# ConsenSys/wittgenstein

Hardware: NVIDIA H100
Metric: simulated-ms/sec, GSFSignature 65,536 nodes (higher is better)
Workload: dtype u64 bitmaps / int32

## Files before the change

wittgenstein_b200/csrc/wtg_cuda.cu:

```cuda
#include <cuda_runtime.h>
#include <unistd.h>

#include <cstdio>
#include <cstdlib>
#include <stdexcept>
#include <string>
#include <vector>

#include "wtg_engine.hpp"

namespace wtg {

#define CUDA_OK(x)                                                                                       \
  do {                                                                                                   \
    cudaError_t e_ = (x);                                                                                \
    if (e_ != cudaSuccess) throw std::runtime_error(std::string("CUDA: ") + cudaGetErrorString(e_) + " at " #x); \
  } while (0)

constexpr int SCAN_THREADS = 256;
constexpr int SCAN_ITEMS = 4;
constexpr int SCAN_TILE = SCAN_THREADS * SCAN_ITEMS;

__global__ void k_begin(Dev d, int mode) {
  if (threadIdx.x >= 32) return;
// ... 424 lines not shown
  if (warp >= 4) return;
  const int gw = blk * 4 + warp, nw = nBlk * 4;
  CoopWarp c;
  for (int k = gw; k < cnt; k += nw) xBuildAll(d, c, k, d.allTmp + (size_t)gw * d.N, hist[warp]);
}

constexpr int MS_SUB = 256;
constexpr int MS_ROUNDS = MS_SUB / 32;
__device__ __forceinline__ void msZero(int* hist, int ring, int warps) {
  for (int i = threadIdx.x * 4; i < warps * ring; i += blockDim.x * 4) *reinterpret_cast<int4*>(hist + i) = make_int4(0, 0, 0, 0);
}
__device__ __forceinline__ void msWarpHistogram(const Dev& d, int* hw, int g0, int G, int tick, int lane, int (&tg)[MS_ROUNDS]) {
#pragma unroll
  for (int r = 0; r < MS_ROUNDS; ++r) {
    int g = g0 + r * 32 + lane;
    tg[r] = g < G ? d.newTarget[g] : -1;
  }
#pragma unroll
  for (int r = 0; r < MS_ROUNDS; ++r)
    if (tg[r] >= 0) atomicAdd(&hw[tg[r] - tick], 1);
}
__global__ void __launch_bounds__(256) k_ms_count(Dev d) {
  extern __shared__ int msHist[];
  if (d.ctl->error) return;
  const int blk = blockIdx.x, nBlk = gridDim.x;
  const int G = d.ctl->totalSlots, tick = d.ctl->tick, ring = d.ring;
  const int W = d.msWarps, CH = W * MS_SUB;
  const int nChunks = (G + CH - 1) / CH;
  const int warp = threadIdx.x >> 5, lane = threadIdx.x & 31;
  for (int ch = blk; ch < nChunks; ch += nBlk) {
    msZero(msHist, ring, W);
    __syncthreads();
    int tg[MS_ROUNDS];
    msWarpHistogram(d, msHist + warp * ring, ch * CH + warp * MS_SUB, G, tick, lane, tg);
    __syncthreads();
    int* row = d.msCount + (size_t)ch * ring;
    for (int b = threadIdx.x; b < ring; b += blockDim.x) {
      int tot = 0;
      for (int w = 0; w < W; ++w) tot += msHist[w * ring + b];
      row[b] = tot;
    }
    __syncthreads();
  }
}
__global__ void k_ms_scan(Dev d) {
  if (d.ctl->error) return;
  const int blk = blockIdx.x, nBlk = gridDim.x;
  int G = d.ctl->totalSlots, tick = d.ctl->tick, ring = d.ring;
  const int CH = d.msWarps * MS_SUB;
  int nChunks = (G + CH - 1) / CH;
  if (nChunks == 0) return;
  for (int b = blk * blockDim.x + threadIdx.x; b < ring; b += nBlk * blockDim.x) {
    int slot = (tick + b) & (ring - 1);
    int run = d.bucketCount[slot];
    for (int ch0 = 0; ch0 < nChunks; ch0 += 8) {
      int v[8];
#pragma unroll
      for (int k = 0; k < 8; ++k) v[k] = ch0 + k < nChunks ? d.msCount[(size_t)(ch0 + k) * ring + b] : 0;
#pragma unroll
      for (int k = 0; k < 8; ++k)
        if (ch0 + k < nChunks) {
          d.msCount[(size_t)(ch0 + k) * ring + b] = run;
          run += v[k];
        }
    }
    if (run > d.bcap) {
      setError(d, ERR_BUCKET_OVERFLOW, tick + b);
      run = d.bcap;
    }
    d.bucketCount[slot] = run;
  }
}
__global__ void __launch_bounds__(256) k_ms_scatter(Dev d) {
  extern __shared__ int msHist[];
  if (d.ctl->error) return;
  const int blk = blockIdx.x, nBlk = gridDim.x;
  const int G = d.ctl->totalSlots, tick = d.ctl->tick, ring = d.ring;
  const int W = d.msWarps, CH = W * MS_SUB;
  const int nChunks = (G + CH - 1) / CH;
  const int warp = threadIdx.x >> 5, lane = threadIdx.x & 31;
  int* base = msHist + warp * ring;
  CoopWarp cw;
  for (int ch = blk; ch < nChunks; ch += nBlk) {
    msZero(msHist, ring, W);
    __syncthreads();
    const int g0 = ch * CH + warp * MS_SUB;
    int tg[MS_ROUNDS];
    msWarpHistogram(d, base, g0, G, tick, lane, tg);
    __syncthreads();
    const int* row = d.msCount + (size_t)ch * ring;
    for (int b = threadIdx.x; b < ring; b += blockDim.x) {
      int run = row[b];
      for (int w = 0; w < W; ++w) {
        int c = msHist[w * ring + b];
        msHist[w * ring + b] = run;
        run += c;
      }
    }
    __syncthreads();
#pragma unroll
    for (int r = 0; r < MS_ROUNDS; ++r) {
      int g = g0 + r * 32 + lane;
      int t = tg[r];
      int pos = cw.claim(base, t - tick, t >= 0);
      if (t >= 0) {
        if (pos < d.bcap) {
          const int4* src = reinterpret_cast<const int4*>(d.newEv + g);
          int4* dst = reinterpret_cast<int4*>(d.buckets + (size_t)(t & (ring - 1)) * (size_t)d.bcap + pos);
          int4 x = src[0], y = src[1];
          dst[0] = x;
          dst[1] = y;
          if (d.G > 1) d.bucketKey[(size_t)(t & (ring - 1)) * (size_t)d.bcap + pos] = orderKey((unsigned)d.ctl->xseq, (unsigned)g);
        }
        if (d.G > 1) d.newTarget[g] = -1;
      }
      __syncwarp();
    }
    __syncthreads();
  }
}

__global__ void k_free(Dev d) {
  if (d.ctl->error) return;
  const int blk = blockIdx.x, nBlk = gridDim.x;
  const int per = d.freeCap / ARENA_STRIPES;
  const int stripe = blk & (ARENA_STRIPES - 1);
  int cnt = d.ctl->freeCnt[stripe];
  if (cnt > per) cnt = per;
  const int sub = (blk >> 6) * blockDim.x + threadIdx.x;
  const int nsub = (nBlk >> 6) * blockDim.x;
  for (int j = sub; j < cnt; j += nsub) freeApply(d, stripe * per + j);
}

__global__ void k_gsf_init_nodes(Dev d) {
  int n = d.n0 + blockIdx.x * blockDim.x + threadIdx.x;
  if (n < d.n0 + d.nLoc) gsfInitNodeBody(d, n);
}
__global__ void k_rng_candidates(Dev d, u64 s0, u64 count, u64 chunk, int maxBound, u64* out, int* outCount, int cap) {
  u64 t = (u64)blockIdx.x * blockDim.x + threadIdx.x;
  u64 start = t * chunk;
  if (start >= count) return;
  u64 len = start + chunk <= count ? chunk : count - start;
  rngCandidateChunk(d, s0, start, len, maxBound, out, outCount, cap);
}
template <class PeerT>
__global__ void k_gsf_shuffle(Dev d, int l, u64 s0, const int* liveRank, const u64* rejOrd, int nRej) {
  int n = d.n0 + blockIdx.x * blockDim.x + threadIdx.x;
  if (n < d.n0 + d.nLoc) gsfShuffleLevel<PeerT>(d, n, l, s0, liveRank, rejOrd, nRej);
}

class CudaBackend : public Backend {
 public:
  cudaStream_t st = nullptr;
  int devId = 0;
  void bind() const { cudaSetDevice(devId); }
  int sms = 132;
  int smemOptin = 0;
  cudaGraphExec_t tickGraph = nullptr;
  const void* graphFor = nullptr;
  bool useGraph = true;
  long long launches = 0;
  long long graphKernels = 0;
  cudaEvent_t tm0 = nullptr, tm1 = nullptr;
  enum ProfSlot { P_BEGIN, P_COND_SCAN, P_DISPATCH_COUNT, P_SCAN_PARTIAL, P_EXCHANGE, P_SCAN_FINAL, P_DISPATCH_SCATTER, P_NODE,
                  P_EMIT, P_MS_COUNT, P_MS_SCAN, P_MS_SCATTER, P_FREE, P_END, P_COND_SCORE, P_COND_SELECT, NK };
  bool profiling = false;
  std::vector<cudaEvent_t> evPool;
  std::vector<int> evKernel;
  size_t evUsed = 0;
  double profMs[NK] = {};
  long long profCnt[NK] = {};
  const char* profNames[NK] = {"k_begin", "k_cond_scan", "k_dispatch_count", "k_scan_partial", "k_exchange", "k_scan_final",
                               "k_dispatch_scatter", "k_node", "k_emit", "k_ms_count", "k_ms_scan", "k_ms_scatter", "k_free",
                               "k_end", "k_cond_score", "k_cond_select"};

  explicit CudaBackend(int requested = -1) {
    int dev = 0;
    const char* e = std::getenv("LOCAL_RANK");
    int cnt = 0;
    CUDA_OK(cudaGetDeviceCount(&cnt));
    if (cnt == 0) throw std::runtime_error("no CUDA device");
    if (e) dev = std::atoi(e) % cnt;
    const char* e2 = std::getenv("WTG_DEVICE");
    if (e2) dev = std::atoi(e2) % cnt;
    if (requested >= 0) {
      if (requested >= cnt) throw std::invalid_argument("CUDA device " + std::to_string(requested) + " does not exist");
      dev = requested;
    }
    CUDA_OK(cudaSetDevice(dev));
    devId = dev;
    cudaDeviceProp p;
    CUDA_OK(cudaGetDeviceProperties(&p, dev));
    sms = p.multiProcessorCount;
    CUDA_OK(cudaStreamCreateWithFlags(&st, cudaStreamNonBlocking));
    CUDA_OK(cudaDeviceGetAttribute(&smemOptin, cudaDevAttrMaxSharedMemoryPerBlockOptin, dev));
    CUDA_OK(cudaFuncSetAttribute(k_ms_count, cudaFuncAttributeMaxDynamicSharedMemorySize, smemOptin));
    CUDA_OK(cudaFuncSetAttribute(k_ms_scatter, cudaFuncAttributeMaxDynamicSharedMemorySize, smemOptin));
    const char* g = std::getenv("WTG_NO_GRAPH");
    if (g && g[0] == '1') useGraph = false;
  }
  ~CudaBackend() override {
    for (void* q : ipcOpened) cudaIpcCloseMemHandle(q);
    if (tickGraph) cudaGraphExecDestroy(tickGraph);
    if (st) cudaStreamDestroy(st);
  }
  void* alloc(size_t bytes) override {
    bind();
    void* p = nullptr;
    cudaError_t e = cudaMalloc(&p, bytes);
    if (e != cudaSuccess) throw std::runtime_error("cudaMalloc of " + std::to_string(bytes) + " bytes failed: " + cudaGetErrorString(e));
    CUDA_OK(cudaMemsetAsync(p, 0, bytes, st));
    return p;
  }
  void release(void* p) override { cudaFree(p); }
  int deviceId() const override { return devId; }
  void exportShared(void* p, unsigned char* handle) override {
    bind();
    std::memset(handle, 0, 128);
    cudaIpcMemHandle_t ih;
    CUDA_OK(cudaIpcGetMemHandle(&ih, p));
    static_assert(sizeof(ih) == 64, "cudaIpcMemHandle_t");
    std::memcpy(handle, &ih, 64);
    long long pid = (long long)getpid();
    std::memcpy(handle + 64, &pid, 8);
    std::memcpy(handle + 72, &p, sizeof(p));
    std::memcpy(handle + 80, &devId, 4);
  }
  std::vector<void*> ipcOpened;
  void* importShared(const unsigned char* handle) override {
    bind();
    long long pid;
    void* p;
    int dev;
    std::memcpy(&pid, handle + 64, 8);
    std::memcpy(&p, handle + 72, sizeof(p));
    std::memcpy(&dev, handle + 80, 4);
    if (pid == (long long)getpid()) {
      if (dev != devId) {
        int can = 0;
        CUDA_OK(cudaDeviceCanAccessPeer(&can, devId, dev));
        if (!can) throw std::runtime_error("GPU " + std::to_string(devId) + " cannot access GPU " + std::to_string(dev) + " (peer access)");
        cudaError_t e = cudaDeviceEnablePeerAccess(dev, 0);
        if (e != cudaSuccess && e != cudaErrorPeerAccessAlreadyEnabled) CUDA_OK(e);
        cudaGetLastError();
      }
      return p;
    }
    cudaIpcMemHandle_t ih;
    std::memcpy(&ih, handle, 64);
    void* q = nullptr;
    CUDA_OK(cudaIpcOpenMemHandle(&q, ih, cudaIpcMemLazyEnablePeerAccess));
    ipcOpened.push_back(q);
    return q;
  }
  void upload(void* dst, const void* src, size_t bytes) override {
    bind();
    CUDA_OK(cudaMemcpyAsync(dst, src, bytes, cudaMemcpyHostToDevice, st));
    CUDA_OK(cudaStreamSynchronize(st));
  }
  void download(void* dst, const void* src, size_t bytes) override {
    bind();
    CUDA_OK(cudaMemcpyAsync(dst, src, bytes, cudaMemcpyDeviceToHost, st));
    CUDA_OK(cudaStreamSynchronize(st));
  }
  void sync() override {
    bind();
    CUDA_OK(cudaStreamSynchronize(st));
    drainProfile();
  }
  void timerStart() override {
    bind();
    if (!tm0) {
      CUDA_OK(cudaEventCreate(&tm0));
      CUDA_OK(cudaEventCreate(&tm1));
    }
    CUDA_OK(cudaEventRecord(tm0, st));
  }
  double timerStopMs() override {
    bind();
    CUDA_OK(cudaEventRecord(tm1, st));
    CUDA_OK(cudaEventSynchronize(tm1));
    float ms = 0;
    CUDA_OK(cudaEventElapsedTime(&ms, tm0, tm1));
    return (double)ms;
  }
  void profileEnable(bool on) override {
    sync();
    profiling = on;
    if (on) {
      for (int i = 0; i < NK; ++i) {
        profMs[i] = 0;
        profCnt[i] = 0;
      }
    }
  }
  int profileRead(double* ms, long long* cnt, const char** names, int cap) override {
    sync();
    int k = 0;
    for (int i = 0; i < NK && k < cap; ++i, ++k) {
      ms[k] = profMs[i];
      cnt[k] = profCnt[i];
      names[k] = profNames[i];
    }
    return k;
  }
  void drainProfile() {
    for (size_t i = 0; i < evUsed; ++i) {
      float ms = 0;
      cudaEventElapsedTime(&ms, evPool[2 * i], evPool[2 * i + 1]);
      profMs[evKernel[i]] += ms;
      profCnt[evKernel[i]] += 1;
    }
    evUsed = 0;
  }
  void profBegin(int kid) {
    if (!profiling) return;
    if (evUsed * 2 + 2 > evPool.size()) {
      if (evUsed >= 8192) {
        CUDA_OK(cudaStreamSynchronize(st));
        drainProfile();
      } else {
        cudaEvent_t a, b;
        CUDA_OK(cudaEventCreate(&a));
        CUDA_OK(cudaEventCreate(&b));
        evPool.push_back(a);
        evPool.push_back(b);
        evKernel.push_back(0);
      }
    }
    evKernel[evUsed] = kid;
    CUDA_OK(cudaEventRecord(evPool[2 * evUsed], st));
  }
  void profEnd() {
    if (!profiling) return;
    CUDA_OK(cudaEventRecord(evPool[2 * evUsed + 1], st));
    ++evUsed;
  }

  void enqueueTick(const Dev& d, int mode) {
    const int wide = sms * 8;
    const size_t msSmem = (size_t)d.msWarps * d.ring * sizeof(int);
    if (mode != 3) {
      profBegin(P_BEGIN);
      k_begin<<<1, 32, 0, st>>>(d, mode);
      profEnd();
    }
    if ((d.proto == PROTO_GSF || d.proto == PROTO_HANDEL) && mode != 3) {
      const size_t smem8 = d.proto == PROTO_GSF ? (size_t)8 * (size_t)(d.qcap / 32) * sizeof(uint32_t) : 0;
      profBegin(P_COND_SCAN);
      k_cond_mark<<<(d.nLoc + 255) / 256, 256, 0, st>>>(d);
      k_cond_nodes<0><<<ARENA_STRIPES * 19, 256, 0, st>>>(d);
      profEnd();
      profBegin(P_COND_SCORE);
      k_cond_score<<<ARENA_STRIPES * 19, 256, 0, st>>>(d);
      profEnd();
      profBegin(P_COND_SELECT);
      k_cond_nodes<1><<<ARENA_STRIPES * 19, 256, smem8, st>>>(d);
      profEnd();
      launches += 4;
      if (d.proto == PROTO_HANDEL) {
        profBegin(P_SCAN_PARTIAL);
        k_scan_partial<<<wide, SCAN_THREADS, 0, st>>>(d, 2);
        profEnd();
        profBegin(P_SCAN_FINAL);
        k_scan_final<<<wide, SCAN_THREADS, 0, st>>>(d, 2);
        profEnd();
        if (d.G > 1) {
          profBegin(P_EXCHANGE);
          k_hpick_publish<<<sms, 256, 0, st>>>(d);
          k_x_sync<<<1, 32, 0, st>>>(d, 3);
          profEnd();
          profBegin(P_COND_SELECT);
          k_hpick_xcheck<<<sms, 256, 0, st>>>(d);
          k_hpick_xapply<<<sms, 256, 0, st>>>(d);
          profEnd();
          launches += 5;
        } else {
          profBegin(P_COND_SELECT);
          k_hpick_check<<<sms, 256, 0, st>>>(d);
          k_hpick_apply<<<sms, 256, 0, st>>>(d);
          profEnd();
          launches += 3;
        }
      }
    }
    if (mode != 2 && mode != 3) {
      profBegin(P_DISPATCH_COUNT);
      k_dispatch_count<<<wide, 256, 0, st>>>(d);
      profEnd();
      profBegin(P_SCAN_PARTIAL);
      k_scan_partial<<<wide, SCAN_THREADS, 0, st>>>(d, 0);
      profEnd();
      profBegin(P_SCAN_FINAL);
      k_scan_final<<<wide, SCAN_THREADS, 0, st>>>(d, 0);
      profEnd();
      profBegin(P_DISPATCH_SCATTER);
      k_dispatch_scatter<<<wide, 256, 0, st>>>(d);
      profEnd();
      profBegin(P_NODE);
      k_node_msgs<<<(d.nLoc + 255) / 256, 256, 0, st>>>(d);
      k_node_tasks<<<ARENA_STRIPES * 19, 256, 0, st>>>(d);
      if (d.proto == PROTO_CASPER) {
        k_casper_fixups<<<1, 32, 0, st>>>(d);
        launches += 1;
      }
      profEnd();
      launches += 6;
    }
    profBegin(P_SCAN_PARTIAL);
    k_scan_partial<<<wide, SCAN_THREADS, 0, st>>>(d, 1);
    profEnd();
    profBegin(P_SCAN_FINAL);
    k_scan_final<<<wide, SCAN_THREADS, 0, st>>>(d, 1);
    profEnd();
    if (d.G > 1) {
      profBegin(P_EXCHANGE);
      k_x1_publish<<<sms * 2, 256, 0, st>>>(d);
      k_x_sync<<<1, 32, 0, st>>>(d, 0);
      k_x1_totals<<<1, 1, 0, st>>>(d);
      k_x1_offsets<<<sms * 2, 256, 0, st>>>(d);
      profEnd();
      launches += 4;
    }
    profBegin(P_EMIT);
    if (d.shufCap > 0) {
      k_shuffle_check<<<ARENA_STRIPES * 4, 256, 0, st>>>(d);
      k_shuffle_serial<<<1, 1, 0, st>>>(d);
      launches += 2;
    }
    k_emit<<<ARENA_STRIPES * 16, 256, 0, st>>>(d);
    if (d.allCap > 0) {
      if (d.G > 1)
        k_x_all_publish<<<8, 128, 0, st>>>(d);
      else
        k_emit_all<<<d.allWarps / 4, 128, 0, st>>>(d);
      launches += 1;
    }
    profEnd();
    if (d.G > 1) {
      profBegin(P_EXCHANGE);
      k_x_sync<<<1, 32, 0, st>>>(d, 1);
      k_x2_ingest<<<sms * 4, 256, 0, st>>>(d);
      launches += 2;
      if (d.allCap > 0) {
        k_x_all_build<<<d.allWarps / 4, 128, 0, st>>>(d);
        launches += 1;
      }
      profEnd();
    }
    profBegin(P_MS_COUNT);
    k_ms_count<<<sms * 2, d.msWarps * 32, msSmem, st>>>(d);
    profEnd();
    profBegin(P_MS_SCAN);
    k_ms_scan<<<(d.ring + 127) / 128, 128, 0, st>>>(d);
    profEnd();
    profBegin(P_MS_SCATTER);
    k_ms_scatter<<<sms * 2, d.msWarps * 32, msSmem, st>>>(d);
    profEnd();
    const bool pooled = d.proto == PROTO_GSF || d.proto == PROTO_HANDEL;
    if (pooled) {
      profBegin(P_FREE);
      k_free<<<ARENA_STRIPES * 2, 256, 0, st>>>(d);
      profEnd();
    }
    profBegin(P_END);
    k_end<<<1, 1, 0, st>>>(d, mode);
    profEnd();
    launches += pooled ? 9 : 8;
  }
  void configure(const Dev& d) {
    const size_t msSmem = (size_t)d.msWarps * d.ring * sizeof(int);
    if (msSmem > (size_t)smemOptin) throw std::runtime_error("time ring too large for the multisplit's shared-memory histogram");
  }
  void tick(const Dev& d, int mode) override {
    bind();
    configure(d);
    enqueueTick(d, mode);
    CUDA_OK(cudaGetLastError());
  }
  void ticks(const Dev& d, int count) override {
    bind();
    configure(d);
    if (!useGraph || profiling || count < 4) {
      for (int i = 0; i < count; ++i) enqueueTick(d, 1);
      CUDA_OK(cudaGetLastError());
      return;
    }
    if (!tickGraph || graphFor != (const void*)d.ctl) {
      if (tickGraph) cudaGraphExecDestroy(tickGraph);
      cudaGraph_t g;
      long long before = launches;
      CUDA_OK(cudaStreamBeginCapture(st, cudaStreamCaptureModeThreadLocal));
      enqueueTick(d, 1);
      CUDA_OK(cudaStreamEndCapture(st, &g));
      graphKernels = launches - before;
      launches = before;
      CUDA_OK(cudaGraphInstantiate(&tickGraph, g, 0));
      cudaGraphDestroy(g);
      graphFor = (const void*)d.ctl;
    }
    for (int i = 0; i < count; ++i) CUDA_OK(cudaGraphLaunch(tickGraph, st));
    launches += graphKernels * count;
  }
  void gsfInitNodes(const Dev& d) override {
    bind();
    k_gsf_init_nodes<<<(d.nLoc + 255) / 256, 256, 0, st>>>(d);
    CUDA_OK(cudaGetLastError());
  }
  void rngCandidates(const Dev& d, unsigned long long s0, unsigned long long count, int maxBound,
                     std::vector<unsigned long long>& out) override {
    bind();
    const u64 chunk = 16384;
    u64 threads = (count + chunk - 1) / chunk;
    int cap = (int)std::min<u64>((u64)1 << 26, count / 1024 + (1 << 16));
    u64* dOut = nullptr;
    int* dCnt = nullptr;
    CUDA_OK(cudaMalloc(&dOut, (size_t)cap * sizeof(u64)));
    CUDA_OK(cudaMalloc(&dCnt, sizeof(int)));
    CUDA_OK(cudaMemsetAsync(dCnt, 0, sizeof(int), st));
    u64 blocks = (threads + 127) / 128;
    k_rng_candidates<<<(unsigned)blocks, 128, 0, st>>>(d, s0, count, chunk, maxBound, dOut, dCnt, cap);
    CUDA_OK(cudaGetLastError());
    int n = 0;
    CUDA_OK(cudaMemcpyAsync(&n, dCnt, sizeof(int), cudaMemcpyDeviceToHost, st));
    CUDA_OK(cudaStreamSynchronize(st));
    if (n > cap) {
      cudaFree(dOut);
      cudaFree(dCnt);
      throw std::runtime_error("rng candidate list overflow");
    }
    out.resize((size_t)n);
    if (n) CUDA_OK(cudaMemcpyAsync(out.data(), dOut, (size_t)n * sizeof(u64), cudaMemcpyDeviceToHost, st));
    CUDA_OK(cudaStreamSynchronize(st));
    cudaFree(dOut);
    cudaFree(dCnt);
  }
  void gsfShufflePeers(const Dev& d, unsigned long long s0, const int* liveRank, const unsigned long long* rejOrd, int nRej) override {
    bind();
    for (int l = d.L - 1; l >= 1; --l) {
      if (d.peerBits == 16)
        k_gsf_shuffle<uint16_t><<<(d.nLoc + 127) / 128, 128, 0, st>>>(d, l, s0, liveRank, rejOrd, nRej);
      else
        k_gsf_shuffle<uint32_t><<<(d.nLoc + 127) / 128, 128, 0, st>>>(d, l, s0, liveRank, rejOrd, nRej);
    }
    CUDA_OK(cudaGetLastError());
    CUDA_OK(cudaStreamSynchronize(st));
  }
};

Backend* makeBackend(int device) { return new CudaBackend(device); }
long long backendLaunches(Backend* b) { return static_cast<CudaBackend*>(b)->launches; }

}

#define WTG_API(name) wtg_##name
#include "wtg_capi.inl"
```

wittgenstein_b200/csrc/wtg_engine.hpp:

```cpp
#pragma once
#include <chrono>
#include <cstdio>
#include <functional>
#include <thread>
#include <cstdlib>
#include <cstring>
#include <memory>
#include <string>
#include <vector>

#include "wtg_host.hpp"
#include "wtg_logic.cuh"
#include "wtg_types.h"

namespace wtg {

struct GsfParams {
  int nodeCount, threshold, pairingTime, timeoutPerLevelMs, periodDurationMs, acceleratedCallsCount, nodesDown;
};

struct SfParams {
  int nodeCount, threshold, pairingTime, signatureSize, replyTimeout, candidateCount;
};

// ... 658 lines not shown
    d.sfP = P;
    d.sfThreshold = sp.threshold;
    d.sfPairing = sp.pairingTime;
    d.sfSigSize = sp.signatureSize;
    d.sfReplyTimeout = sp.replyTimeout;
    d.sfCandCount = sp.candidateCount;
    std::vector<int> cpl(N, P), agg(N, 1);
    d.sfCpl = dupload(cpl);
    d.sfAgg = dupload(agg);
    d.sfFlags = dalloc<int>(N);
    d.sfThresholdAt = dalloc<long long>(N);
    d.sfSentReq = dalloc<int>(N);
    d.sfRecvReq = dalloc<int>(N);
    d.sfCacheMask = dalloc<uint32_t>(N);
    d.sfCache = dalloc<int>((size_t)N * 32);
    d.sfUsedWords = std::max(1, N / 128);
    d.sfUsedBits = dalloc<unsigned long long>((size_t)N * d.sfUsedWords);
    d.sfPendBits = dalloc<unsigned long long>((size_t)N * d.sfUsedWords);
    d.shufCap = d.newEvCap;
    d.forceShufSerial = forceShufSerial ? 1 : 0;
    d.byG = dalloc<int>(d.newEvCap);
    {
      std::vector<int> m1((size_t)d.newEvCap, -1);
      d.byGTick = dupload(m1);
    }
    d.descDraw = dalloc<int>(d.descCap);
    std::vector<Ev> tasks((size_t)N);
    for (int i = 0; i < N; ++i) {
      Ev ev;
      std::memset(&ev, 0, sizeof(ev));
      ev.pad = 1;
      ev.kind = EV_TASK;
      ev.to = (uint32_t)i;
      ev.from = (uint32_t)i;
      ev.meta = SF_T_GO;
      tasks[(size_t)i] = ev;
    }
    if (N > d.bcap) throw std::runtime_error("bucket capacity too small");
    be->upload(d.buckets + (size_t)1 * d.bcap, tasks.data(), tasks.size() * sizeof(Ev));
    be->upload(d.bucketCount + 1, &N, sizeof(int));
    Ctl c;
    std::memset(&c, 0, sizeof(c));
    c.callId = 1;
    c.rng = hm.rd.seed;
    writeCtl(c);
    inited = true;
  }

  HandelParams hp{};
  void handelInit(const HandelParams& p) {
    requireNotInited();
    const int N = p.nodeCount;
    if (p.nodesDown >= N || p.nodesDown < 0 || p.threshold > N || (p.nodesDown + p.threshold > N))
      throw std::invalid_argument("nodeCount=" + std::to_string(N) + ", threshold=" + std::to_string(p.threshold));
    if (N < 2 || (N & (N - 1)) != 0) throw std::invalid_argument("We support only power of two nodes in this simulation");
    if (p.byzantineSuicide && p.hiddenByzantine) throw std::invalid_argument("Only one attack at a time");
    if (p.fastPath < 0 || p.fastPath > MAX_ACC) throw std::invalid_argument("fastPath must be in [0,16]");
    if (p.disseminationPeriodMs <= 0 || p.pairingTime < 0 || p.desynchronizedStart < 0) throw std::invalid_argument("period/pairing/desynchronizedStart");
    checkLatencyBuilder();
    hp = p;
    std::vector<char> bad((size_t)N, 0);
    for (int setDown = 0; setDown < p.nodesDown;) {
      int down = hm.rd.nextInt(N);
      if (down != 1 && !bad[(size_t)down]) {
        bad[(size_t)down] = 1;
        setDown++;
      }
    }
    std::vector<int> startAt((size_t)N, 0);
    for (int i = 0; i < N; ++i) {
      startAt[(size_t)i] = p.desynchronizedStart == 0 ? 0 : hm.rd.nextInt(p.desynchronizedStart);
      hm.buildNodes(1);
      if (bad[(size_t)i]) hm.nodes[(size_t)i].down = true;
    }
    int L = 1;
    while ((1 << L) <= N) ++L;
    if (sharded()) {
      const long long nl = N / shardWorld;
      long long words = 0;
      for (int l = INLINE_MAX_LEVEL + 1; l < L; ++l)
        if ((1LL << (l - 1)) >= nl) words += (1LL << (l - 1)) / 64;
      stageWordsWanted = std::max<long long>(65536, nl * words + 8192);
      if (tun.stageWords) stageWordsWanted = tun.stageWords;
      xProtoBytes = hPickBytes(shardWorld, (int)nl);
    }
    allocCommon(N, PROTO_HANDEL);
    for (int i = 0; i < N; ++i)
      if (startAt[(size_t)i] + 1 >= d.ring) throw std::invalid_argument("desynchronizedStart exceeds the time ring");
    const int NL = d.nLoc, n0 = d.n0;
    d.L = L;
    d.W64 = std::max(1, N / 64);
    d.threshold = p.threshold;
    d.period = p.disseminationPeriodMs;
    d.hLevelWait = p.levelWaitTime;
    d.hFastPath = p.fastPath;
    d.hExtraCycle = p.extraCycle;
    d.hByzSuicide = p.byzantineSuicide;
    d.hWinInit = 16;
    d.hWinMin = 1;
    d.hWinMax = 128;
    d.qcap = (int)(tun.qcap ? tun.qcap : std::min<long long>(4096, std::max<long long>(64, 2LL * N)));
    d.qcap = (d.qcap + 31) / 32 * 32;
    const size_t W = (size_t)d.W64;
    {
      std::vector<unsigned long long> diag((size_t)NL * W, 0);
      for (int i = n0; i < n0 + NL; ++i) diag[(size_t)(i - n0) * W + (size_t)(i >> 6)] = 1ULL << (i & 63);
      for (unsigned long long** row : {&d.hLastAgg, &d.hTotInc, &d.hVerInd}) {
        *row = dallocNodes<unsigned long long>(W);
        be->upload(*row + (size_t)n0 * W, diag.data(), diag.size() * sizeof(unsigned long long));
      }
    }
    d.hToVerInd = dallocNodes<unsigned long long>(W);
    d.hFinPeers = dallocNodes<unsigned long long>(W);
    d.hBlack = dallocNodes<unsigned long long>(W);
    std::vector<int> zerosNL((size_t)N * L, 0), outFin((size_t)N * L, 0), biz((size_t)N * L, p.byzantineSuicide ? 0 : -1), cnt0((size_t)N * L, 0);
    std::vector<uint32_t> ver((size_t)N * L, 1);
    for (int i = 0; i < N; ++i) {
      outFin[(size_t)i * L] = 1;
      cnt0[(size_t)i * L] = 1;
    }
    d.hPos = duploadNodes(zerosNL, L);
    d.hOutFin = duploadNodes(outFin, L);
    d.hBiz = duploadNodes(biz, L);
    {
      std::vector<int> nohit((size_t)N * L, -2147483647 - 1);
      d.hBizNoHit = duploadNodes(nohit, L);
    }
    d.hCntLast = duploadNodes(cnt0, L);
    d.hCntInc = duploadNodes(cnt0, L);
    d.hCntInd = duploadNodes(cnt0, L);
    d.lvVer = duploadNodes(ver, L);
    std::vector<int> ones((size_t)N, 1), win((size_t)N, d.hWinInit), added((size_t)N, p.extraCycle), pairing((size_t)N), minStart((size_t)N);
    for (int i = 0; i < N; ++i) {
      pairing[(size_t)i] = (int)std::max(1.0, p.pairingTime * hm.nodes[(size_t)i].speed);
      minStart[(size_t)i] = startAt[(size_t)i] + 1;
    }
    d.hTotal = duploadNodes(ones);
    d.hWindow = duploadNodes(win);
    d.hAddedCycle = duploadNodes(added);
    d.pairing = duploadNodes(pairing);
    d.minStart = duploadNodes(minStart);
    d.stamp = dallocNodes<uint32_t>();
    d.hStartAt = duploadNodes(startAt);
    d.hSigsChecked = dallocNodes<int>();
    d.hSigQueueSize = dallocNodes<int>();
    d.hMsgFiltered = dallocNodes<int>();
    d.hSeq = dallocNodes<int>();
    d.qLen = dallocNodes<int>();
    d.hQueue = dallocNodes<HQEntry>((size_t)d.qcap);
    d.qStamp = dallocNodes<uint32_t>((size_t)d.qcap);
    d.hCand = dallocNodes<int>(32);
    d.hCandK = dallocNodes<int>();
    d.hDrawBase = dallocNodes<int>();
    d.hHidden = p.hiddenByzantine ? 1 : 0;
    d.forcePickSerial = forcePickSerial ? 1 : 0;
    d.hbNoPeers = dallocNodes<int>();
    {
      std::vector<int> m1((size_t)N, -1);
      d.hbLastId = duploadNodes(m1);
    }
    d.hbLastFrom = dallocNodes<int>();
    const bool timing_ = std::getenv("WTG_INIT_TIMING") != nullptr;
    auto t0_ = std::chrono::steady_clock::now();
    auto lap_ = [&](const char* what) {
      if (!timing_) return;
      auto t1 = std::chrono::steady_clock::now();
      std::fprintf(stderr, "[handel init] %s: %.2f s\n", what, std::chrono::duration<double>(t1 - t0_).count());
      t0_ = t1;
    };
    lap_("nodes + rows");
    unsigned hw = std::thread::hardware_concurrency();
    int T = (int)std::max(1u, std::min(hw ? hw : 1u, 64u));
    if (N < 2048) T = 1;
    auto parallelFor = [&](int n, const std::function<void(int, int)>& body) {
      if (T == 1) {
        body(0, n);
        return;
      }
      std::vector<std::thread> th;
      int per = (n + T - 1) / T;
      for (int t = 0; t < T; ++t) {
        int b0 = t * per, b1 = std::min(n, b0 + per);
        if (b0 < b1) th.emplace_back(body, b0, b1);
      }
      for (auto& x : th) x.join();
    };
    std::vector<int> ranksOwn((size_t)NL * N);
    std::unique_ptr<int[]> ranksT_(new int[(size_t)N * N]);
    int* const ranksT = ranksT_.get();
    {
      std::vector<int> expected((size_t)N);
      for (int i = 0; i < N; ++i) expected[(size_t)i] = i;
      const int RB = std::min(N, 1024);
      std::vector<int> blk((size_t)RB * N);
      for (int r0 = 0; r0 < N; r0 += RB) {
        const int r1 = std::min(N, r0 + RB);
        for (int n = r0; n < r1; ++n) {
          for (int i = N; i > 1; --i) std::swap(expected[(size_t)i - 1], expected[(size_t)hm.rd.nextInt(i)]);
          int* row = blk.data() + (size_t)(n - r0) * N;
          for (int i = 0; i < N; ++i) row[expected[(size_t)i]] = i;
        }
        for (int n = std::max(r0, n0); n < std::min(r1, n0 + NL); ++n)
          std::memcpy(ranksOwn.data() + (size_t)(n - n0) * N, blk.data() + (size_t)(n - r0) * N, sizeof(int) * (size_t)N);
        parallelFor(N, [&](int c0, int c1) {
          for (int c = c0; c < c1; ++c) {
            int* dst = ranksT + (size_t)c * N + r0;
            for (int r = r0; r < r1; ++r) dst[r - r0] = blk[(size_t)(r - r0) * N + c];
          }
        });
      }
    }
    lap_("reception ranks");
    std::vector<uint32_t> peersOwn((size_t)NL * (size_t)(N - 1), 0);
    {
      struct Run {
        uint32_t off, len;
      };
      const int CH = std::min(N, 16 * T);
      std::vector<std::vector<Run>> runs((size_t)CH);
      auto ownList = [&](int sIdx) { return sIdx >= n0 && sIdx < n0 + NL ? peersOwn.data() + (size_t)(sIdx - n0) * (size_t)(N - 1) : nullptr; };
      auto sortSender = [&](int sIdx, std::vector<unsigned long long>& keys, std::vector<Run>& rs) {
        rs.clear();
        if (hm.nodes[(size_t)sIdx].down) return;
        const int* col = ranksT + (size_t)sIdx * N;
        uint32_t* list = ownList(sIdx);
        for (int l = 1; l < L; ++l) {
          Blk wb = levelBlock(sIdx ^ (1 << (l - 1)), l);
          keys.resize((size_t)wb.size);
          for (int i = 0; i < wb.size; ++i)
            keys[(size_t)i] = ((unsigned long long)(uint32_t)col[wb.base + i] << 32) | (unsigned long long)(uint32_t)(wb.base + i);
          std::sort(keys.begin(), keys.end());
          const uint32_t lo = (1u << (l - 1)) - 1u;
          if (list)
            for (int i = 0; i < wb.size; ++i) list[lo + (uint32_t)i] = (uint32_t)(keys[(size_t)i] & 0xFFFFFFFFULL);
          for (int i = 0; i < wb.size;) {
            int j = i + 1;
            while (j < wb.size && (keys[(size_t)j] >> 32) == (keys[(size_t)i] >> 32)) ++j;
            if (j - i > 1) rs.push_back(Run{lo + (uint32_t)i, (uint32_t)(j - i)});
            i = j;
          }
        }
      };
      for (int c0 = 0; c0 < N; c0 += CH) {
        const int c1 = std::min(N, c0 + CH);
        parallelFor(c1 - c0, [&](int a, int b) {
          std::vector<unsigned long long> keys;
          for (int i = a; i < b; ++i) sortSender(c0 + i, keys, runs[(size_t)i]);
        });
        for (int sIdx = c0; sIdx < c1; ++sIdx) {
          uint32_t* list = ownList(sIdx);
          for (const Run& r : runs[(size_t)(sIdx - c0)])
            for (int m = (int)r.len; m > 1; --m) {
              const int j = hm.rd.nextInt(m);
              if (list) std::swap(list[r.off + (uint32_t)m - 1], list[r.off + (uint32_t)j]);
            }
        }
      }
    }
    lap_("emission lists");
    ranksT_.reset();
    {
      int* pr = dalloc<int>((size_t)NL * N);
      be->upload(pr, ranksOwn.data(), ranksOwn.size() * sizeof(int));
      d.hRanks = pr - (size_t)n0 * N;
      uint32_t* pp = dalloc<uint32_t>((size_t)NL * (size_t)(N - 1));
      be->upload(pp, peersOwn.data(), peersOwn.size() * sizeof(uint32_t));
      d.peers = pp - (size_t)n0 * (size_t)(N - 1);
    }
    d.peerBits = 32;
    lap_("upload");
    Ctl c;
    std::memset(&c, 0, sizeof(c));
    long long perNode = tun.poolSlotsPerNode ? tun.poolSlotsPerNode : 24;
    for (int l = INLINE_MAX_LEVEL + 1; l < L; ++l) {
      long long slots = std::max<long long>(1024, perNode * NL);
      slots = (slots + POOL_STRIPES - 1) / POOL_STRIPES * POOL_STRIPES;
      d.poolCap[l] = (int)slots;
      d.pool[l] = dalloc<unsigned long long>((size_t)slots * (size_t)poolWords(l));
      d.poolRef[l] = dalloc<int>((size_t)slots);
      std::vector<uint32_t> fl((size_t)slots);
      long long per = slots / POOL_STRIPES;
      for (int sidx = 0; sidx < POOL_STRIPES; ++sidx) {
        for (long long i = 0; i < per; ++i) fl[(size_t)(sidx * per + i)] = (uint32_t)(sidx * per + (per - 1 - i));
        c.poolFreeCnt[l][sidx] = (int)per;
      }
      d.poolFree[l] = dupload(fl);
      c.poolMinFree[l] = (int)slots;
    }
    std::vector<std::vector<Ev>> per((size_t)d.ring);
    std::vector<std::vector<unsigned long long>> perKey((size_t)d.ring);
    for (int i = n0; i < n0 + NL; ++i)
      if (!hm.nodes[(size_t)i].down) {
        Ev ev;
        std::memset(&ev, 0, sizeof(ev));
        ev.pad = 1;
        ev.kind = EV_PERIODIC;
        ev.to = (uint32_t)i;
        ev.from = (uint32_t)i;
        per[(size_t)(startAt[(size_t)i] + 1)].push_back(ev);
        perKey[(size_t)(startAt[(size_t)i] + 1)].push_back(orderKey(0, (unsigned)i));
      }
    for (int t = 0; t < d.ring; ++t)
      if (!per[(size_t)t].empty()) {
        if ((int)per[(size_t)t].size() > d.bcap) throw std::runtime_error("bucket capacity too small");
        be->upload(d.buckets + (size_t)t * d.bcap, per[(size_t)t].data(), per[(size_t)t].size() * sizeof(Ev));
        if (sharded()) be->upload(d.bucketKey + (size_t)t * d.bcap, perKey[(size_t)t].data(), perKey[(size_t)t].size() * sizeof(unsigned long long));
// ... 615 lines not shown
```

wittgenstein_b200/csrc/wtg_types.h:

```cpp
#pragma once
#include <stdint.h>

#if defined(__CUDACC__)
#define WTG_HD __host__ __device__ __forceinline__
#else
#define WTG_HD inline
#endif

namespace wtg {

constexpr int POOL_STRIPES = 64;
constexpr int ARENA_STRIPES = 64;
constexpr int MS_SUB_ENVELOPES = 256;
constexpr int MAX_LEVELS = 24;
constexpr int MAX_ACC = 16;
constexpr int INLINE_MAX_LEVEL = 7;
constexpr int MAX_DIST = 1144;
constexpr int MAX_SHARDS = 8;

enum : int { PROTO_NONE = 0, PROTO_PINGPONG = 1, PROTO_GSF = 2, PROTO_SANFERMIN = 3, PROTO_HANDEL = 4, PROTO_CASPER = 5, PROTO_CAPPOS = 6 };

enum : uint32_t {
  EV_MSG = 0,
  EV_MULTI = 1,
// ... 241 lines not shown
  int16_t* nextra;
  uint8_t* ncity;
  uint8_t* ndown;
  uint8_t* npart;
  long long* msgReceived;
  long long* msgSent;
  long long* bytesSent;
  long long* bytesReceived;
  long long* doneAt;
  const int16_t* latTab;
  const int16_t* latBase;
  const int16_t* latJit;
  const unsigned long long* jumpA;
  const unsigned long long* jumpC;
  Ev* buckets;
  int* bucketCount;
  int* inboxCnt;
  int* inboxOff;
  int* inboxFill;
  int* nodeTasks;
  int* dueList;
  int* taskList;
  unsigned long long* taskWord;
  int listStripeCap;
  unsigned long long* inbox;
  int* subCount;
  int* itemBase;
  int* evSlots;
  int* evDraws;
  int* condDue;
  uint32_t* workList;
  int* condFired;
  int* condDraws;
  Ev* condEv;
  int* condTarget;
  int* slotBase;
  int* drawBase;
  int* scanPartial;
  Desc* desc;
  uint32_t* destScratch;
  Ev* newEv;
  int* newTarget;
  int* msCount;
  MultiRec* rec;
  uint32_t* recDest;
  int* recArrival;
  uint32_t* freeList;
  int ffwd;
  int farCap;
  FarEv* far;
  int* farSel;
  int allCap;
  int* allList;
  int* allTmp;
  int allWarps;
  int recSlots;
  int shufCap;
  int forceShufSerial;
  int* byG;
  int* byGTick;
  int* descDraw;
  int* pong;
  int cCycle, cBpCount, cAttPerRound, cAttCount, cBlockTime, cAttTime, cRandomTies, cByzDelay;
  int cMaxBlocks, cMaxAtts, cAttWords, cBlkWords, cFirstAtt;
  CasperG* cg;
  uint8_t* cKind;
  int* cHead;
  int* cVotes;
  unsigned long long* cAttRecv;
  unsigned long long* cBlkRecv;
  unsigned long long* cToReeval;
  int* cbHeight;
  int* cbParent;
  int* cbProducer;
  int* cbTime;
  unsigned long long* cbIncluded;
  int* attHead;
  int* attHeight;
  int* cbItem;
  unsigned long long* cbTmp;
  int* cbTmpRow;
  int* cTieItem;
  int* cTieCnt;
  int* cTieList;
  int hLevelWait, hFastPath, hExtraCycle, hByzSuicide, hWinInit, hWinMin, hWinMax;
  unsigned long long* hLastAgg;
  unsigned long long* hTotInc;
  unsigned long long* hVerInd;
  unsigned long long* hToVerInd;
  unsigned long long* hFinPeers;
  unsigned long long* hBlack;
  int* hPos;
  int* hOutFin;
  int* hBiz;
  int* hBizNoHit;
  int* hCntLast;
  int* hCntInc;
  int* hCntInd;
  int* hTotal;
  int* hWindow;
  int* hAddedCycle;
  int* hSigsChecked;
  int* hSigQueueSize;
  int* hMsgFiltered;
  int* hStartAt;
  int* hSeq;
  int* hRanks;
  HQEntry* hQueue;
  int* hCand;
  int* hCandK;
  int* hDrawBase;
  int hHidden;
  int* hbNoPeers;
  int* hbLastId;
  int* hbLastFrom;
  int* poolRef[MAX_LEVELS];
  int sfThreshold, sfPairing, sfSigSize, sfReplyTimeout, sfCandCount, sfP;
  int* sfCpl;
  int* sfAgg;
  int* sfFlags;
  long long* sfThresholdAt;
  int* sfSentReq;
  int* sfRecvReq;
  uint32_t* sfCacheMask;
  int* sfCache;
  int sfTimeout;
  int sfUsedWords;
  unsigned long long* sfUsedBits;
  unsigned long long* sfPendBits;
  unsigned long long* verified;
  unsigned long long* indivSeen;
  unsigned long long* indivVer;
  int* pos;
  int* remaining;
  int* cntVer;
  int* cntIndiv;
  int* cntUnion;
  int* totalCard;
  int* minStart;
  uint32_t* stamp;
  int* pairing;
  int* qLen;
  int* sigChecked;
  int* sigQueueSize;
  QEntry* queue;
  int* qScore;
  uint32_t* qStamp;
  uint32_t* lvVer;
  void* peers;
  unsigned long long* pool[MAX_LEVELS];
  uint32_t* poolFree[MAX_LEVELS];
  int poolCap[MAX_LEVELS];
  int forcePickSerial;
};

}
```

Before: 4666.

## Fork dispatch and free kernels onto a side stream to overlap condition scan

Adds a second stream with fork/join events so that, in mode 1 on a single GPU with GSF or Handel and profiling off, the dispatch count/scan/scatter chain runs concurrently with the condition scoring/selection kernels. The pool-free kernel likewise overlaps the multisplit kernels. Handel's draw scan gets a separate partial buffer so its scan does not race with the dispatch scan's scratch. This cuts serialized small-kernel latency inside the captured tick graph, at the risk of hidden data races between branches.

```diff
diff --git a/wittgenstein_b200/csrc/wtg_cuda.cu b/wittgenstein_b200/csrc/wtg_cuda.cu
--- a/wittgenstein_b200/csrc/wtg_cuda.cu
+++ b/wittgenstein_b200/csrc/wtg_cuda.cu
@@ -600,6 +600,8 @@
 class CudaBackend : public Backend {
  public:
   cudaStream_t st = nullptr;
+  cudaStream_t side = nullptr;
+  cudaEvent_t forkEv = nullptr, joinEv = nullptr;
   int devId = 0;
   void bind() const { cudaSetDevice(devId); }
   int sms = 132;
@@ -641,6 +643,9 @@
     CUDA_OK(cudaGetDeviceProperties(&p, dev));
     sms = p.multiProcessorCount;
     CUDA_OK(cudaStreamCreateWithFlags(&st, cudaStreamNonBlocking));
+    CUDA_OK(cudaStreamCreateWithFlags(&side, cudaStreamNonBlocking));
+    CUDA_OK(cudaEventCreateWithFlags(&forkEv, cudaEventDisableTiming));
+    CUDA_OK(cudaEventCreateWithFlags(&joinEv, cudaEventDisableTiming));
     CUDA_OK(cudaDeviceGetAttribute(&smemOptin, cudaDevAttrMaxSharedMemoryPerBlockOptin, dev));
     CUDA_OK(cudaFuncSetAttribute(k_ms_count, cudaFuncAttributeMaxDynamicSharedMemorySize, smemOptin));
     CUDA_OK(cudaFuncSetAttribute(k_ms_scatter, cudaFuncAttributeMaxDynamicSharedMemorySize, smemOptin));
@@ -650,6 +655,9 @@
   ~CudaBackend() override {
     for (void* q : ipcOpened) cudaIpcCloseMemHandle(q);
     if (tickGraph) cudaGraphExecDestroy(tickGraph);
+    if (forkEv) cudaEventDestroy(forkEv);
+    if (joinEv) cudaEventDestroy(joinEv);
+    if (side) cudaStreamDestroy(side);
     if (st) cudaStreamDestroy(st);
   }
   void* alloc(size_t bytes) override {
@@ -785,14 +793,25 @@
     ++evUsed;
   }
 
+  void fork() {
+    CUDA_OK(cudaEventRecord(forkEv, st));
+    CUDA_OK(cudaStreamWaitEvent(side, forkEv, 0));
+  }
+  void join() {
+    CUDA_OK(cudaEventRecord(joinEv, side));
+    CUDA_OK(cudaStreamWaitEvent(st, joinEv, 0));
+  }
   void enqueueTick(const Dev& d, int mode) {
     const int wide = sms * 8;
     const size_t msSmem = (size_t)d.msWarps * d.ring * sizeof(int);
+    const bool branches = mode == 1 && !profiling && d.G == 1 && (d.proto == PROTO_GSF || d.proto == PROTO_HANDEL);
+    cudaStream_t sd = branches ? side : st;
     if (mode != 3) {
       profBegin(P_BEGIN);
       k_begin<<<1, 32, 0, st>>>(d, mode);
       profEnd();
     }
+    if (branches) fork();
     if ((d.proto == PROTO_GSF || d.proto == PROTO_HANDEL) && mode != 3) {
       const size_t smem8 = d.proto == PROTO_GSF ? (size_t)8 * (size_t)(d.qcap / 32) * sizeof(uint32_t) : 0;
       profBegin(P_COND_SCAN);
@@ -807,11 +826,13 @@
       profEnd();
       launches += 4;
       if (d.proto == PROTO_HANDEL) {
+        Dev dd = d;
+        dd.scanPartial = d.drawScanPartial;
         profBegin(P_SCAN_PARTIAL);
-        k_scan_partial<<<wide, SCAN_THREADS, 0, st>>>(d, 2);
+        k_scan_partial<<<wide, SCAN_THREADS, 0, st>>>(dd, 2);
         profEnd();
         profBegin(P_SCAN_FINAL);
-        k_scan_final<<<wide, SCAN_THREADS, 0, st>>>(d, 2);
+        k_scan_final<<<wide, SCAN_THREADS, 0, st>>>(dd, 2);
         profEnd();
         if (d.G > 1) {
           profBegin(P_EXCHANGE);
@@ -834,17 +855,18 @@
     }
     if (mode != 2 && mode != 3) {
       profBegin(P_DISPATCH_COUNT);
-      k_dispatch_count<<<wide, 256, 0, st>>>(d);
+      k_dispatch_count<<<wide, 256, 0, sd>>>(d);
       profEnd();
       profBegin(P_SCAN_PARTIAL);
-      k_scan_partial<<<wide, SCAN_THREADS, 0, st>>>(d, 0);
+      k_scan_partial<<<wide, SCAN_THREADS, 0, sd>>>(d, 0);
       profEnd();
       profBegin(P_SCAN_FINAL);
-      k_scan_final<<<wide, SCAN_THREADS, 0, st>>>(d, 0);
+      k_scan_final<<<wide, SCAN_THREADS, 0, sd>>>(d, 0);
       profEnd();
       profBegin(P_DISPATCH_SCATTER);
-      k_dispatch_scatter<<<wide, 256, 0, st>>>(d);
-      profEnd();
+      k_dispatch_scatter<<<wide, 256, 0, sd>>>(d);
+      profEnd();
+      if (branches) join();
       profBegin(P_NODE);
       k_node_msgs<<<(d.nLoc + 255) / 256, 256, 0, st>>>(d);
       k_node_tasks<<<ARENA_STRIPES * 19, 256, 0, st>>>(d);
@@ -896,6 +918,7 @@
       }
       profEnd();
     }
+    if (branches) fork();
     profBegin(P_MS_COUNT);
     k_ms_count<<<sms * 2, d.msWarps * 32, msSmem, st>>>(d);
     profEnd();
@@ -908,9 +931,10 @@
     const bool pooled = d.proto == PROTO_GSF || d.proto == PROTO_HANDEL;
     if (pooled) {
       profBegin(P_FREE);
-      k_free<<<ARENA_STRIPES * 2, 256, 0, st>>>(d);
-      profEnd();
-    }
+      k_free<<<ARENA_STRIPES * 2, 256, 0, sd>>>(d);
+      profEnd();
+    }
+    if (branches) join();
     profBegin(P_END);
     k_end<<<1, 1, 0, st>>>(d, mode);
     profEnd();
diff --git a/wittgenstein_b200/csrc/wtg_engine.hpp b/wittgenstein_b200/csrc/wtg_engine.hpp
--- a/wittgenstein_b200/csrc/wtg_engine.hpp
+++ b/wittgenstein_b200/csrc/wtg_engine.hpp
@@ -834,6 +834,7 @@
     d.hCand = dallocNodes<int>(32);
     d.hCandK = dallocNodes<int>();
     d.hDrawBase = dallocNodes<int>();
+    d.drawScanPartial = dalloc<int>(2 * 8192);
     d.hHidden = p.hiddenByzantine ? 1 : 0;
     d.forcePickSerial = forcePickSerial ? 1 : 0;
     d.hbNoPeers = dallocNodes<int>();
diff --git a/wittgenstein_b200/csrc/wtg_types.h b/wittgenstein_b200/csrc/wtg_types.h
--- a/wittgenstein_b200/csrc/wtg_types.h
+++ b/wittgenstein_b200/csrc/wtg_types.h
@@ -417,6 +417,7 @@
   uint32_t* poolFree[MAX_LEVELS];
   int poolCap[MAX_LEVELS];
   int forcePickSerial;
+  int* drawScanPartial;
 };
 
 }
```

Result: faster. 4974 (median of 6 runs) (+6.6%).
